# c5shen/WITCH

Measured on AMD Instinct MI355X. Metric: query-seqs aligned/sec (100k queries x 200-HMM eHMM), higher is better.
Workload: dtype f32; 1 GPU; dna_100k_x200; n_queries=100000, n_hmms=200, query_len=150, model_len_min=898, model_len_max=993, k=10, pairs_reported_rank0=20000000, pairs_multidomain_rank0=968, pairs_long_list_rank0=0, pairs_dense_redo_rank0=3, topk_crc32=3263627139

## Files before the change

include/witch_hip.h:

```cpp
#ifndef WITCH_HIP_H
#define WITCH_HIP_H

#include <stdint.h>

#ifdef __cplusplus
extern "C" {
#endif

#define WH_OK          0
#define WH_EINVAL     -1
#define WH_EIO        -2
#define WH_ENODEV     -3
#define WH_EHIP       -4
#define WH_ERANGE     -5
#define WH_ENOMEM     -6

#define WH_ALPH_DNA    0
#define WH_ALPH_RNA    1
#define WH_ALPH_AMINO  2

#define WH_FLAG_REPORTED  1
#define WH_FLAG_MULTI     2
#define WH_FLAG_OVERRIDE  4
#define WH_FLAG_TRUNC     8
// ... 113 lines not shown
int wh_filter_host(const char *const *hmm_paths, int n, const uint8_t *residues, const int64_t *offsets, int64_t nq,
                   const wh_filter_opts *opts, uint8_t *stage, float *filter_bias_nats, int32_t *msv_raw, int32_t *vit_raw,
                   int64_t *counts4);
int wh_score_filtered(wh_ehmm *e, const uint8_t *residues, const int64_t *offsets, int64_t nq, const wh_filter_opts *opts,
                      int32_t *decibits, uint8_t *flags, float *fwd_bits, wh_pair_detail *detail, uint8_t *stage);
int wh_score_filtered_dev(wh_ehmm *e, const uint8_t *d_residues, const int64_t *d_offsets, int64_t nq, int64_t total_residues,
                          int32_t max_len, const wh_filter_opts *opts, int32_t *d_decibits, uint8_t *d_flags, float *d_fwd_bits,
                          wh_pair_detail *d_detail, uint8_t *d_stage, void *stream);
int wh_last_filter_counts(wh_ehmm *e, int64_t out[6]);

int wh_last_align_status(wh_ehmm *e, int64_t *n_logspace, int64_t *n_unaligned, int64_t *unaligned_pairs, int64_t cap);

int wh_last_align_paths(wh_ehmm *e, int64_t *paths4);

int wh_last_score_paths(wh_ehmm *e, int64_t *paths6);
int wh_last_score_counters(wh_ehmm *e, int64_t *out8);
int wh_last_region_overflow(wh_ehmm *e, int64_t *out4);
int wh_last_long_query_pairs(wh_ehmm *e, int64_t out[2]);
int wh_last_long_score_pairs(wh_ehmm *e, int64_t out[2]);
int wh_last_long_align_pairs(wh_ehmm *e, int64_t out[2]);

int wh_set_path_buffer(wh_ehmm *e, uint8_t *d_paths);
int wh_set_path_buffer16(wh_ehmm *e, uint16_t *d_paths);

int wh_last_queue_reruns(wh_ehmm *e);

int wh_consensus(wh_ehmm *e, const int64_t *offsets, int64_t nq, const int64_t *qpair_off,
                 const int32_t *pair_h, const double *pair_w, const int64_t *col_offsets, const int32_t *cols,
                 const int64_t *ret_off, const int32_t *retained, const int32_t *nongaps,
                 int32_t backbone_length, int32_t *out, int32_t *minmax);
// ... 79 lines not shown
```

witch_amd/_lib.py:

```python
from __future__ import annotations

import ctypes as C
import os
import subprocess

_HERE = os.path.dirname(os.path.abspath(__file__))
LIB_PATH = os.path.join(_HERE, "libwitch_hip.so")
CSRC = os.path.join(_HERE, "csrc")

WH_MAX_ENVELOPES = 16
FLAG_REPORTED, FLAG_MULTI, FLAG_OVERRIDE, FLAG_TRUNC, FLAG_EXACT = 1, 2, 4, 8, 16
FLAG_FILTERED = 32
STAGE_MSV, STAGE_BIAS, STAGE_VIT, STAGE_VIT_RAN, STAGE_FWD = 1, 2, 4, 8, 16
VIT_NOT_RUN, VIT_OVERFLOW, MSV_OVERFLOW = -32769, 32768, -1
ALPH_DNA, ALPH_RNA, ALPH_AMINO = 0, 1, 2
WH_OK, WH_EINVAL, WH_EIO, WH_ENODEV, WH_EHIP, WH_ERANGE, WH_ENOMEM = 0, -1, -2, -3, -4, -5, -6
WH_BUILD_STATS, WH_BUILD_CALIB_NO_LDS = 1, 4
WH_MSA_TRIM, WH_MSA_NO_LDS, WH_MSA_CONS_HMMER = 1, 2, 4
PATH_P2_WIN, PATH_P2_FULL, PATH_P4_W256, PATH_P4_W512, PATH_P4_WFAIL, PATH_P4_FULL, PATH_DENSE, PATH_MULTI = 1, 2, 4, 8, 16, 32, 64, 128


class WitchHipError(RuntimeError):
    pass

# ... 88 lines not shown
                                  C.POINTER(C.c_void_p), C.POINTER(C.c_int64)] + [C.POINTER(C.c_void_p)] * 5 + [_P]),
    "wh_filter": (C.c_int, [_P, _P, _P, C.c_int64, _P, _P, _P, _P, _P]),
    "wh_filter_dev": (C.c_int, [_P, _P, _P, C.c_int64, C.c_int64, C.c_int32, _P, _P, _P, _P, _P, _P]),
    "wh_filter_host": (C.c_int, [C.POINTER(C.c_char_p), C.c_int, _P, _P, C.c_int64, _P, _P, _P, _P, _P, _P]),
    "wh_score_filtered": (C.c_int, [_P, _P, _P, C.c_int64, _P, _P, _P, _P, _P, _P]),
    "wh_score_filtered_dev": (C.c_int, [_P, _P, _P, C.c_int64, C.c_int64, C.c_int32, _P, _P, _P, _P, _P, _P, _P]),
    "wh_last_filter_counts": (C.c_int, [_P, _P]),
    "wh_ehmm_evparams": (C.c_int, [_P, _P, _P, _P]),
    "wh_hmm_evparams": (C.c_int, [C.c_char_p, C.POINTER(C.c_float), C.POINTER(C.c_float), C.POINTER(C.c_int32)]),
    "wh_consensus": (C.c_int, [_P, _P, C.c_int64, _P, _P, _P, _P, _P, _P, _P, _P, C.c_int32, _P, _P]),
    "wh_consensus_dev": (C.c_int, [_P, _P, C.c_int64, C.c_int32, _P, _P, _P, _P, _P, _P, _P, _P, C.c_int32, C.c_int32, _P, _P, _P]),
    "wh_last_align_status": (C.c_int, [_P, C.POINTER(C.c_int64), C.POINTER(C.c_int64), _P, C.c_int64]),
    "wh_last_align_paths": (C.c_int, [_P, _P]),
    "wh_last_score_paths": (C.c_int, [_P, _P]),
    "wh_last_score_counters": (C.c_int, [_P, _P]),
    "wh_set_path_buffer": (C.c_int, [_P, _P]),
    "wh_set_path_buffer16": (C.c_int, [_P, _P]),
    "wh_last_queue_reruns": (C.c_int, [_P]),
    "wh_last_region_overflow": (C.c_int, [_P, _P]),
    "wh_last_long_query_pairs": (C.c_int, [_P, _P]),
    "wh_last_long_score_pairs": (C.c_int, [_P, _P]),
    "wh_last_long_align_pairs": (C.c_int, [_P, _P]),
    "wh_last_score_launches": (C.c_int, [_P, _P, _P, _P, C.c_int]),
    "wh_last_kernel_ms": (C.c_int, [_P, C.c_int, C.POINTER(C.c_double), C.POINTER(C.c_int)]),
    "wh_set_timing": (C.c_int, [_P, C.c_int]),
    "wh_set_option": (C.c_int, [_P, C.c_char_p, C.c_char_p]),
}

_LIB = None

# ... 36 lines not shown
```

witch_amd/csrc/wh_api.hip:

```cpp
#include <atomic>
#include <chrono>
#include <memory>
#include <thread>

#include "wh_host.h"

static int g_device = -1;

extern "C" {

const char *wh_version(void) { return "witch_hip 0.1.0 (gfx950)"; }
const char *wh_last_error(void) { return wh::last_error(); }

int wh_init(int device) {
  int n = 0;
  if (hipGetDeviceCount(&n) != hipSuccess || n <= 0) {
    set_error("no HIP device visible");
    return WH_ENODEV;
  }
  if (device < 0 || device >= n) {
    set_error("device %d out of range (0..%d)", device, n - 1);
    return WH_EINVAL;
  }
  HIPCHK(hipSetDevice(device));
// ... 217 lines not shown

int wh_last_align_paths(wh_ehmm *e, int64_t *paths4) {
  if (!e || !paths4) { set_error("wh_last_align_paths: bad argument"); return WH_EINVAL; }
  for (int t = 0; t < 4; t++) paths4[t] = e->last_align_paths[t];
  return WH_OK;
}

int wh_last_score_paths(wh_ehmm *e, int64_t *paths6) {
  int64_t *paths4 = paths6;
  if (!e || !paths4) { set_error("wh_last_score_paths: bad argument"); return WH_EINVAL; }
  HIPCHK(hipSetDevice(e->device));
  unsigned long long v[6] = {0, 0, 0, 0, 0, 0};
  HIPCHK(hipDeviceSynchronize());
  HIPCHK(hipMemcpy(v, e->counter(kSlotScorePath), sizeof v, hipMemcpyDeviceToHost));
  for (int t = 0; t < 6; t++) paths4[t] = (int64_t)v[t];
  return WH_OK;
}

int wh_last_score_counters(wh_ehmm *e, int64_t *out8) {
  if (!e || !out8) { set_error("wh_last_score_counters: bad argument"); return WH_EINVAL; }
  HIPCHK(hipSetDevice(e->device));
  unsigned long long v[8] = {0, 0, 0, 0, 0, 0, 0, 0};
  HIPCHK(hipDeviceSynchronize());
  HIPCHK(hipMemcpy(v, e->counter(kSlotScorePath), sizeof v, hipMemcpyDeviceToHost));
  for (int t = 0; t < 8; t++) out8[t] = (int64_t)v[t];
  out8[7] = e->last_long_list;
  return WH_OK;
}

int wh_set_path_buffer(wh_ehmm *e, uint8_t *d_paths) {
  if (!e) { set_error("wh_set_path_buffer: null handle"); return WH_EINVAL; }
  e->path_buf = d_paths;
  return WH_OK;
}

int wh_set_path_buffer16(wh_ehmm *e, uint16_t *d_paths) {
  if (!e) { set_error("wh_set_path_buffer16: null handle"); return WH_EINVAL; }
  e->path_buf16 = d_paths;
  return WH_OK;
}
// ... 339 lines not shown
```

witch_amd/csrc/wh_host_score.hip:

```cpp
#include "wh_host.h"

static const int kStagedMaxBatches = 1 << 15;
static const int kStagedQB = 48;

static int resolve_main_cap(int max_M) {
  const size_t per_wave = (kLdsBudget - resolve_lds_header_bytes(0)) / (size_t)resolve_waves_per_cu();
  int lo = 1, hi = 1 << 20;
  while (lo < hi) {
    const int mid = lo + (hi - lo + 1) / 2;
    if (resolve_lds_bytes(mid, max_M) <= per_wave) lo = mid; else hi = mid - 1;
  }
  return lo;
}

static ScoreCall score_call(wh_ehmm *e, const uint8_t *d_residues, const int64_t *d_offsets, int64_t nq, int64_t total_residues, int32_t max_len,
                            int32_t *d_decibits, uint8_t *d_flags, float *d_fwd_bits, wh_pair_detail *d_detail, void *stream) {
  ScoreCall c = {e, (hipStream_t)stream, d_residues, d_offsets, nq, total_residues, max_len, d_decibits, d_flags, d_fwd_bits, d_detail};
  c.Lc = std::max(max_len, 1);
  c.H = (int)e->hmms.size();
  c.npairs_all = nq * (int64_t)c.H;
  const bool fits = resolve_lds_bytes(c.Lc, e->max_M) <= kLdsBudget;
  c.Lmain = fits || e->knobs.no_long_query ? c.Lc : resolve_main_cap(e->max_M);
  c.resolve = !e->knobs.no_resolve && (fits || !e->knobs.no_long_query) && c.npairs_all < 0x7FFFFFFF;
  c.mixed = nq > 0 && total_residues > 0 && (double)max_len > 1.25 * (double)total_residues / (double)nq;
// ... 97 lines not shown
static ScoreArgs class_args(const ScoreCall &c, const ScoreClassPlan &p, int launches) {
  const wh_ehmm *e = c.e;
  const Knobs &kn = e->knobs;
  ScoreArgs a;
  fill_common(a, c);
  a.tables = (const float *)e->d_tables.p;
  a.hmm_list = (const int32_t *)e->d_lists.p + p.list_off; a.n_list = p.n_list;
  a.counter = e->counter(kSlotLaunch0 + launches);
  a.dbg = kn.dbg;
  a.no_window = kn.no_window ? 1 : 0;
  a.keep_scale = kn.keep_scale;
  a.spill_band = kn.kernel != 9 ? kn.spill_band : 0;
  a.Klds = p.Klds; a.SP = p.b.SP; a.wave_lds = p.b.wave_lds; a.spec_arrays = kScoreSpecArrays;
  if (p.family == ScoreFamily::PhaseCall || p.family == ScoreFamily::FourEnvelope) a.spec_arrays |= kScoreSpecLayout << 8;
  a.paths = reinterpret_cast<unsigned long long *>(e->counter(kSlotScorePath));
  a.p2win = p.p2win;
  a.qorder = p.use_qorder ? c.d_qorder : nullptr;
  a.QB = p.QB; a.n_qblocks = p.n_qblocks; a.n_items = p.n_items;
  a.scratch_stride = p.scratch_stride; a.spec_stride = p.spec_stride;
  a.scratch = (float *)e->d_scratch.p;
  if (p.specg) a.spec_scratch = (float *)e->d_spec.p;
  return a;
}

static int print_class_stats(const ScoreCall &c, int Q, const unsigned long long *stats) {
  unsigned long long st[40];
  if (int rc = stats_read(c, stats, st)) return rc;
  const double tot = (double)(st[4] + st[5] + st[6] + st[7] + st[8] + st[9] + st[10] + st[11]);
  fprintf(stderr, "[wh] Q=%d wave cycles: P1 %.1f%%  P2 %.1f%%  regions %.1f%%  P3 %.1f%%  P4 %.1f%%  null2 %.1f%%  swaps+barriers %.1f%%  other %.1f%%  (total %.3g ticks)\n", Q, 100.0 * st[4] / tot,
          100.0 * st[5] / tot, 100.0 * st[6] / tot, 100.0 * st[7] / tot, 100.0 * st[8] / tot, 100.0 * st[9] / tot, 100.0 * st[10] / tot, 100.0 * st[11] / tot, tot);
  if (st[38]) fprintf(stderr, "[wh] Q=%d wave lifetimes %.3g cycles: %.1f%% in the phases above, %.1f%% fetching an item (two barriers)\n", Q, (double)st[38], 100.0 * tot / (double)st[38], 100.0 * (double)st[39] / (double)st[38]);
  if (st[37]) fprintf(stderr, "[wh] Q=%d four-envelope sweeps: %llu envelopes, %.0f wave cycles per envelope (slot 'null2' above)\n", Q, st[37], (double)st[9] / (double)st[37]);
  fprintf(stderr, "[wh] Q=%d envelope Backward sweeps: %llu on a 256-node window, %llu on a 512-node window, %llu windows failed the mass certificate, %llu full width; union of the stored lane blocks: span %.1f blocks (with margin), %.1f blocks set, of %llu envelopes\n", Q, st[0], st[1], st[2], st[3], (double)st[12] / (double)std::max(1ull, st[14]), (double)st[15] / (double)std::max(1ull, st[14]), st[14]);
  fprintf(stderr, "[wh] Q=%d multihit Backward on a window: %llu scans, of them in doubt at a threshold %llu, at the multidomain bound %llu; window loss out of range %llu; mean eps %.3g\n", Q,
          st[35], st[32], st[33], st[36], st[35] ? 1e-9 * (double)st[34] / (double)st[35] : 0.0);
  fprintf(stderr, "[wh] Q=%d |Ld - mass| / Ld  (<3e-7, <1e-6, <3e-6, <1e-5, <2e-5, more): window sweeps %llu %llu %llu %llu %llu %llu; full-width sweeps %llu %llu %llu %llu %llu %llu\n", Q,
          st[16], st[17], st[18], st[19], st[20], st[21], st[22], st[23], st[24], st[25], st[26], st[27]);
  return WH_OK;
}

static int launch_score_class(const ScoreCall &c, const ScoreClassPlan &p, int *launches) {
  wh_ehmm *e = c.e;
  hipStream_t s = c.s;
  const int Q = p.Q, waves = p.b.waves, threads = waves * kWave;
  const bool big = p.family == ScoreFamily::PassSync;
  ScoreArgs a = class_args(c, p, *launches);
  if (a.p2win == 2) {
    a.p2_backup_stride = (size_t)kScoreSpecArrays * a.SP;
    if (e->d_p2bak.ensure((size_t)p.blocks * waves * a.p2_backup_stride * sizeof(float))) return WH_ENOMEM;
    a.p2_backup = (float *)e->d_p2bak.p;
  }
  if (int rc = stats_begin(c, 320, 13, &a.stats)) return rc;
  if (e->knobs.trace) fprintf(stderr, "[wh] score Q=%d kernel=%s specg=%d waves=%d blocks=%d lds=%zu SP=%d wave_lds=%d items=%d Lcap=%d\n", Q,
                              kFamilyName[(int)p.family], (int)p.specg, waves, p.blocks, p.b.lds, a.SP, a.wave_lds, a.n_items, a.Lcap);
  HIPCHK(hipMemsetAsync(a.counter, 0, sizeof(int), s));
  if (class_mark(e, s, Q, big ? 1 : 0)) return WH_EHIP;
  hipError_t err = big ? launch_score_big(Q, a, p.blocks, threads, p.b.lds, s)
                   : p.family == ScoreFamily::TwoQuery ? launch_score9(Q, a, p.blocks, threads, p.b.lds, s)
                   : p.family == ScoreFamily::FourEnvelope ? launch_score7q(Q, a, p.blocks, threads, p.b.lds, s)
                   : p.family == ScoreFamily::PhaseCallB ? launch_score7b(Q, a, p.blocks, threads, p.b.lds, s)
                                                         : launch_score7(Q, a, p.blocks, threads, p.b.lds, s);
  if (err != hipSuccess) { set_error("score kernel launch (Q=%d) failed: %s", Q, hipGetErrorString(err)); return WH_EHIP; }
  (*launches)++;
  return a.stats ? print_class_stats(c, Q, a.stats) : WH_OK;
}

static int print_staged_stats(const ScoreCall &c, int Q, const unsigned long long *stats) {
// ... 355 lines not shown
```

witch_amd/csrc/wh_knobs.h:

```cpp
#pragma once
#include <algorithm>
#include <climits>
#include <cmath>
#include <cstdlib>
#include <cstring>

struct Knobs {
  int kernel = 7;
  float keep_scale = 0.f;
  int spill_band = 1;
  int max_waves = 0;
  bool force_specg = false;
  bool no_logspace = false;
  bool no_wide_align = false;
  bool no_window = false;
  bool no_p2win = false;
  bool no_long_list = false;
  bool no_big_region = false;
  bool no_long_query = false;
  bool no_resolve = false;
  int score_lmain = 0;
  bool no_long_score = false;
  bool longq_force = false;
  int rqueue_cap = 0;
  int item_g = 0;
  int st_units = 0;
  bool stats = false, trace = false;
  int dbg = 0;
  int rdbg = 0;
};

// ... 9 lines not shown
  {"WH_SCORE_KERNEL", true, [](Knobs &k, const char *v) { const int kv = *v ? atoi(v) : 7; if (kv < 7 || kv > 12) return false; k.kernel = kv; return true; }},
  {"WH_KEEP_LOG2", true, [](Knobs &k, const char *v) { k.keep_scale = *v ? ldexpf(1.0f, atoi(v)) : 0.f; return true; }},
  WH_KNOB_INT("WH_SPILL_BAND", false, spill_band, INT_MIN, INT_MAX, 1),
  WH_KNOB_INT("WH_MAX_WAVES", true, max_waves, 1, 16, 0),
  WH_KNOB_BOOL("WH_FORCE_SPECG", force_specg),
  WH_KNOB_BOOL("WH_NO_LOGSPACE", no_logspace),
  WH_KNOB_BOOL("WH_NO_RESOLVE", no_resolve),
  WH_KNOB_BOOL("WH_NO_LONG_LIST", no_long_list),
  WH_KNOB_BOOL("WH_NO_BIG_REGION", no_big_region),
  WH_KNOB_BOOL("WH_NO_LONG_QUERY", no_long_query),
  WH_KNOB_INT("WH_SCORE_LMAIN", true, score_lmain, 0, INT_MAX, 0),
  WH_KNOB_BOOL("WH_NO_LONG_SCORE", no_long_score),
  WH_KNOB_BOOL("WH_LONGQ_FORCE", longq_force),
  WH_KNOB_BOOL("WH_NO_WINDOW", no_window),
  WH_KNOB_BOOL("WH_NO_P2WIN", no_p2win),
  WH_KNOB_INT("WH_RQUEUE_CAP", true, rqueue_cap, 1, INT_MAX, 0),
  WH_KNOB_INT("WH_ITEM_G", true, item_g, 1, 1024, 0),
  WH_KNOB_INT("WH_ST_UNITS", true, st_units, 16, INT_MAX, 0),
  WH_KNOB_BOOL("WH_NO_WIDE_ALIGN", no_wide_align),
  WH_KNOB_BOOL("WH_STATS", stats),
  WH_KNOB_BOOL("WH_TRACE", trace),
  WH_KNOB_INT("WH_DBG", true, dbg, INT_MIN, INT_MAX, 0),
  WH_KNOB_INT("WH_RDBG", true, rdbg, INT_MIN, INT_MAX, 0),
};
#undef WH_KNOB_BOOL
#undef WH_KNOB_INT

static inline int set_knob(Knobs &k, const char *name, const char *value) {
  for (const KnobEntry &kn : kKnobs)
    if (!strcmp(name, kn.name)) return kn.apply(k, value ? value : "") ? 1 : -1;
// ... 3 lines not shown
```

witch_amd/csrc/wh_score7.hip:

```cpp
#include <hip/hip_runtime.h>

#include "wh_device.h"
#include "wh_launch.h"

#ifndef WH_K7NS
#define WH_K7NS k7
#define WH_K7LAUNCH launch_score7
#endif

namespace wh {
namespace WH_K7NS {


constexpr float kKeepScale7 = 5.9604645e-08f;
constexpr float kMassTol7 = 2e-5f;
constexpr float kWinTol7 = 3e-6f;
__device__ __forceinline__ float spill_tol(bool banded) { return banded ? kWinTol7 : kMassTol7; }
#ifndef WH_K7_MAXQP
#define WH_K7_MAXQP 0
#endif
constexpr int kMaxQP = WH_K7_MAXQP;
#ifdef WH_SLIM_SPEC
constexpr bool kSlim = true;
constexpr int kSpML = SP_B, kSpMH = SP_E, kSpArr = 6;
// ... 10 lines not shown
#ifndef WH_SPEC_ROWS
#define WH_SPEC_ROWS WH_K7_NEW_DEFAULT
#endif
#ifndef WH_UNI
#define WH_UNI WH_K7_NEW_DEFAULT
#endif
#ifndef WH_ROW_PAIRS
#define WH_ROW_PAIRS (WH_K7_NEW_DEFAULT ? 3 : 0)
#endif
#ifndef WH_SPLIT_SLACK
#define WH_SPLIT_SLACK 1
#endif
#ifndef WH_ROW_WAITS
#define WH_ROW_WAITS (WH_K7_NEW_DEFAULT ? 3 : 0)
#endif
constexpr int kLayout = WH_SPEC_ROWS ? SPEC_ROWS : SPEC_SOA;
constexpr bool kUni = WH_UNI != 0;
constexpr bool kRowPairs = ((WH_ROW_PAIRS) & 1) != 0, kUniArgs = ((WH_ROW_PAIRS) & 2) != 0, kSplitSlack = WH_SPLIT_SLACK != 0;
constexpr bool kDrain = ((WH_ROW_WAITS) & 1) != 0, kLateRequest = ((WH_ROW_WAITS) & 2) != 0;
static_assert(kLayout == SPEC_SOA || kSlim, "a row record has six words (WH_SLIM_SPEC)");
template <bool SG> using SpecOf = SpecAt<SG ? (int)SPEC_SOA : kLayout>;
constexpr int kSpecTag = kSpArr | (kLayout << 8);

__device__ __noinline__ static double dlog(double x) { return log(x); }
__device__ __noinline__ static double dexp(double x) { return exp(x); }
__device__ __forceinline__ float flogsum0_v7(float b) {
  const float mx = b > 0.f ? b : 0.f, mn = b > 0.f ? 0.f : b;
  if (mn == -INFINITY || (mx - mn) >= 15.7f) return mx;
  const int idx = (int)((mx - mn) * 1000.0f);
  return mx + (float)dlog(1.0 + dexp((double)-idx / 1000.0));
// ... 684 lines not shown
#pragma unroll
      for (int a = 0; a < BW_NARR; a++) T.v[a][p4] = bw4[a * Q4 * kWave + rev];
    }
  }
  const ScanC sc = scan_prepare(lane_product<QB, true>(T, BW_DD));
  const LdsF4 em4L((const float *)c.emL);
  const float4 *em4G = reinterpret_cast<const float4 *>((const float *)c.emG);
  float Mb[QB], Ib[QB];
#pragma unroll
  for (int p = 0; p < QB; p++) { Mb[p] = 0.f; Ib[p] = 0.f; }
  float xC = cm.move, xJ = 0.f, xN = 0.f, xB = 0.f;
  int eb = 0;
  float ratio = 0.f;
  int S_row = 0;
  float E_row = 0.f, B_row = 0.f;
  if (CARRY) { S_row = speci[at(SP_S, L)]; E_row = spec[at(SP_E, L)]; B_row = spec[at(SP_B, L)]; }
#pragma unroll 1
  for (int i = L; i >= 0; i--) {
    asm volatile("" ::: "memory");
    const int S_i = CARRY ? S_row : 0;
    const float E_i = CARRY ? E_row : 0.f, B_i = CARRY ? B_row : 0.f;
    int S_p = 0;
    float N_p = 0.f, J_p = 0.f, C_p = 0.f;
    if (CARRY) {
      const int ip = i >= 1 ? i - 1 : 0;
      S_p = speci[at(SP_S, ip)]; N_p = spec[at(SP_N, ip)]; J_p = spec[at(SP_J, ip)]; C_p = spec[at(SP_C, ip)];
      E_row = spec[at(SP_E, ip)]; B_row = spec[at(SP_B, ip)];
      S_row = S_p;
    }
    if (i < L) {
      const int x = __builtin_amdgcn_readfirstlane((int)seq[i]);
      float part = 0.f;
      auto emit = [&](auto em_ld) {
#pragma unroll
        for (int p4 = 0; p4 < B4; p4++) {
          const float4 E = T.v[BW_E][p4];
          const float4 O = em_ld(p4);
          Mb[4 * p4 + 0] *= O.w; part = fmaf(E.x, Mb[4 * p4 + 0], part);
          Mb[4 * p4 + 1] *= O.z; part = fmaf(E.y, Mb[4 * p4 + 1], part);
          Mb[4 * p4 + 2] *= O.y; part = fmaf(E.z, Mb[4 * p4 + 2], part);
          Mb[4 * p4 + 3] *= O.x; part = fmaf(E.w, Mb[4 * p4 + 3], part);
        }
      };
      if (x < Klds) emit([&](int p4) { return em4L[x * (Q * 16) + fwd[p4]]; });
      else {
        emit([&](int p4) { return em4G[(size_t)x * (Q * 16) + fwd[p4]]; });
// ... 15 lines not shown
      xB *= r; xJ *= r; xC *= r; xN *= r; xE *= r;
      eb += e;
    }
    const float s_i = ldexpf(invZ, (CARRY ? S_i : speci[at(SP_S, i)]) + eb - ef_L);
    const float pe = (CARRY ? E_i : spec[at(SP_E, i)]) * xE * s_i;
    const float pb = (CARRY ? B_i : spec[at(SP_B, i)]) * xB * s_i;
    float njc = 0.f;
    if (i >= 1) {
      const float s_p = ldexpf(invZ, (CARRY ? S_p : speci[at(SP_S, i, 1)]) + eb - ef_L);
      njc = (CARRY ? N_p : spec[at(SP_N, i, 1)]) * xN;
      njc = fmaf(CARRY ? J_p : spec[at(SP_J, i, 1)], xJ, njc);
      njc = fmaf(CARRY ? C_p : spec[at(SP_C, i, 1)], xC, njc);
      njc = njc * cm.loop * s_p;
    } else {
      ratio = (CARRY ? N_p : spec[at(SP_N, 0)]) * xN * s_i;
    }
    __builtin_amdgcn_wave_barrier();
    if (TMPG) { if (lane == 0) { gE[i] = pe; gB[i] = pb; gN[i] = njc; } }
    else if (lane == 0) {
      if (INPL) { specw[at(SP_E, i)] = pe; specw[at(SP_B, i)] = pb; specw[at(SP_N, i)] = njc; }
      else { tmp[i] = pe; tmp[SP + i] = pb; tmp[2 * SP + i] = njc; }
    }
    __builtin_amdgcn_wave_barrier();
  }
  WinDec o;
  o.eps = 1.0f - ratio;
  return o;
}

template <int TH, bool INPL = false, bool TMPG = false>
// ... 268 lines not shown
    slot = __shfl(slot, 0);
    if (slot < a.rcap && lane == 0) {
      ResolveRec *rr = a.rrecs + slot;
      rr->q = qi; rr->h = h; rr->fwdsc = fwdsc; rr->fwd_bits = fwd_bits_out; rr->nreg = nreg; rr->nenv = nenv;
      rr->multi_mask = multi_mask; rr->flags = flags;
      for (int e = 0; e < nenv; e++) { rr->ri[e] = regs[2 * e]; rr->rj[e] = regs[2 * e + 1]; rr->envsc[e] = envres[e]; rr->domcorr[e] = envres[WH_MAX_ENVELOPES + e]; }
    }
  } else assemble_score(L, Ld_tot, seqbias_sum, sum_score, sb2, fwdsc, nullsc, dp, flags, decibits);
  }
}

struct FrontState {
  float eps_prev, eps_prev2;
  unsigned n_pairs_h;
  unsigned n_p2w, n_p2rej;
};
template <int Q, int TH, bool SG, bool TMPG>
__device__ __forceinline__ RegOut score_regions(const ScoreArgs &a, const WaveCtx &c, uint8_t *seq, int *regs, int L, int lane, LenCfg cm, const FwdOut &f1,
                                                FrontState &fs, long long &t_last, glb_f *tmpg = nullptr) {
  const int SP = c.SP;
  bool saved = false;
  RegOut ro;
  bool have_ro = false;
  if constexpr (Q >= 8 && !SG) {
    const bool try_win = fminf(fs.eps_prev, fs.eps_prev2) * (float)L < 0.17f || (fs.n_pairs_h & 15) == 0;
    fs.n_pairs_h++;
    if ((a.p2win == 1 || TMPG) && !a.no_window && try_win) {
      const unsigned *su = reinterpret_cast<const unsigned *>((const float *)c.n2tab) + kUmSlot;
      const unsigned long long um = ((unsigned long long)su[1] << 32) | su[0];
      if (um != 0) {
        int lo = __builtin_ctzll(um), hi = 63 - __builtin_clzll(um);
        lo = lo > 1 ? lo - 2 : 0; hi = hi < 63 ? hi + 1 : 63;
        const int nodes = (hi - lo + 1) * Q;
        WinDec wd;
        wd.eps = 1.0f;
        if (TMPG && nodes <= (Q % 8 == 0 && Q > 8 ? 8 : 4) * kWave) {
          const float *spec = (const float *)c.spec;
          if (kLayout == SPEC_ROWS) {
            for (int u = lane; u < kSpArr * (L + 1); u += kWave) __builtin_nontemporal_store(spec[u], tmpg + u);
          } else {
            for (int arr = 0; arr < kSpArr; arr++)
              for (int u = lane; u <= L; u += kWave) __builtin_nontemporal_store(spec[arr * SP + u], tmpg + arr * SP + u);
          }
          saved = true;
        }
        if (nodes <= 4 * kWave) wd = sweep_backward_decode_win<4, Q, TH, TMPG, false, false>(c, (lds_u8 *)seq, L, cm, 1.0f / (f1.xC * cm.move), f1.ef, min((63 - hi) * Q, kWave * (Q - 4)));
        else if (Q % 8 == 0 && Q > 8 && nodes <= 8 * kWave) wd = sweep_backward_decode_win<(Q % 8 == 0 ? 8 : 4), Q, TH, TMPG, false, false>(c, (lds_u8 *)seq, L, cm, 1.0f / (f1.xC * cm.move), f1.ef, min((63 - hi) * Q, kWave * (Q - 8)));
        if (nodes <= (Q % 8 == 0 && Q > 8 ? 8 : 4) * kWave) { fs.eps_prev2 = fs.eps_prev; fs.eps_prev = fabsf(wd.eps); }
        if (wd.eps > -1e-4f && wd.eps < 0.01f) {
          ro = region_scan_cert<TH, TMPG, false>(c.spec, SP, L, (lds_i *)regs, lane, fmaxf(wd.eps, 0.f));
          have_ro = ((ro.flags >> 24) & 3) == 0;
          if (a.stats && lane == 0) {
            if ((ro.flags >> 24) & 1) atomicAdd(a.stats + 32, 1ull);
            if ((ro.flags >> 25) & 1) atomicAdd(a.stats + 33, 1ull);
            atomicAdd(a.stats + 34, (unsigned long long)(wd.eps * 1e9f));
            atomicAdd(a.stats + 35, 1ull);
          }
          ro.flags &= 0xFFFFFF;
        } else if (a.stats && lane == 0) atomicAdd(a.stats + 36, 1ull);
        if (have_ro) fs.n_p2w++; else fs.n_p2rej++;
      }
    }
  }
  if (!have_ro) {
    if (TMPG && saved) {
      __builtin_amdgcn_fence(__ATOMIC_SEQ_CST, "workgroup");
      float *spec = (float *)c.spec;
      __builtin_amdgcn_wave_barrier();
      if (kLayout == SPEC_ROWS) {
        for (int u = lane; u < kSpArr * (L + 1); u += kWave) spec[u] = __builtin_nontemporal_load(tmpg + u);
      } else {
        for (int arr = 0; arr < kSpArr; arr++)
          for (int u = lane; u <= L; u += kWave) spec[arr * SP + u] = __builtin_nontemporal_load(tmpg + arr * SP + u);
      }
      __builtin_amdgcn_wave_barrier();
// ... 26 lines not shown

template <int Q, int TH, bool SG>
__global__ __launch_bounds__(TH) void score_kernel7(ScoreArgs a) {
  extern __shared__ __attribute__((aligned(16))) float smem_raw[];
  volatile int *s_item_p = reinterpret_cast<volatile int *>(smem_raw);
  float *smem = smem_raw + 4;
  const int lane = threadIdx.x & 63, wave = __builtin_amdgcn_readfirstlane((int)(threadIdx.x >> 6)), nwaves = blockDim.x >> 6;
  constexpr int TBL = Q * kWave;
  float *emL = smem;
  float *trL = smem + (size_t)a.K * TBL;
  constexpr int NARR = FW_NARR + (Q <= kMaxQP ? 1 : 0);
  float *wbase = trL + 2 * NARR * TBL + (size_t)wave * a.wave_lds;
  const int SP = a.SP;
  WaveCtx c;
  c.emL = (lds_f *)emL; c.fwL = (lds_f *)trL; c.bwL = (lds_f *)(trL + NARR * TBL);
  const int spArrAll = kSpArr + (a.p2win == 1 ? 3 : 0);
  c.spec = (lds_f *)wbase; c.n2tab = (lds_f *)(wbase + (SG ? 0 : spArrAll * SP));
  c.specg = SG ? (glb_f *)(a.spec_scratch + ((size_t)blockIdx.x * nwaves + wave) * a.spec_stride) : nullptr;
  c.degen = 0;
  for (int t = 0; t < 32; t++) if (t == lane) c.degen = a.degen[t];
  c.Fs = (glb_f *)(a.scratch + ((size_t)blockIdx.x * nwaves + wave) * a.scratch_stride);
  c.SP = SP; c.alpha = a.K | (a.Kp << 8) | (a.K << 16); c.lane = lane;
  int *regs = reinterpret_cast<int *>(wbase + (SG ? 0 : spArrAll * SP) + 32);
  uint8_t *seq = reinterpret_cast<uint8_t *>(regs + kRegsInts);
  const double LOG2 = 0.69314718055994529;
  int cur_h = -1;
  const DevHMM *hm = nullptr;
  EnvCounters ec = {0, 0, 0, 0, 0};
  FrontState fs = {0.f, 0.f, 0u, 0u, 0u};

  for (;;) {
    __syncthreads();
    if (threadIdx.x == 0) { *s_item_p = atomicAdd(a.counter, 1); s_item_p[1] = 0; }
    __syncthreads();
    const int item = __builtin_amdgcn_readfirstlane(*s_item_p);
    if (item >= a.n_items) break;
    const int h = __builtin_amdgcn_readfirstlane(a.hmm_list[item / a.n_qblocks]);
    const int64_t q_lo = (int64_t)(item % a.n_qblocks) * a.QB;
    const int64_t q_hi = q_lo + a.QB < a.nq ? q_lo + a.QB : a.nq;
    if (h != cur_h) {
      hm = a.hmms + h;
      const float4 *src = reinterpret_cast<const float4 *>(a.tables + hm->em_off);
      float4 *dst = reinterpret_cast<float4 *>(emL);
      for (int t = threadIdx.x; t < a.K * TBL / 4; t += blockDim.x) dst[t] = src[t];
// ... 60 lines not shown
        a.flags[out] = (uint8_t)flags;
        if (a.fwd_bits) a.fwd_bits[out] = fwd_bits_out;
      }
      const unsigned band_ev = take_band_events(ec);
      if (uint16_t *rec = path_record(a)) {
        if (lane == 0) rec[out] = (uint16_t)path_bits(regs, ec, fs, isfinite(fwd_bits_out), flags, (flags & WH_FLAG_MULTI) && a.rrecs != nullptr, band_ev);
      }
    }
  }
  if (a.paths && lane == 0) {
    if (ec.n_w256) atomicAdd(a.paths + 0, (unsigned long long)ec.n_w256);
    if (ec.n_w512) atomicAdd(a.paths + 1, (unsigned long long)ec.n_w512);
    if (ec.n_wfail) atomicAdd(a.paths + 2, (unsigned long long)ec.n_wfail);
    if (ec.n_full) atomicAdd(a.paths + 3, (unsigned long long)ec.n_full);
    if (ec.spill) atomicAdd(a.paths + 6, ec.spill);
    if (fs.n_p2w) atomicAdd(a.paths + 4, (unsigned long long)fs.n_p2w);
    if (fs.n_p2rej) atomicAdd(a.paths + 5, (unsigned long long)fs.n_p2rej);
  }
}

enum { QR_QLO = 0, QR_QHI, QR_L, QR_NREG, QR_FLAGS, QR_FWDSC, QR_NULLSC, QR_FWDBITS, QR_ENVSC, QR_RI, QR_RJ, QR_XC3, QR_EF3, QR_BAND, QR_INTS = 16 };
template <int Q, int TH>
__global__ __launch_bounds__(TH) void score_kernel7q(ScoreArgs a) {
  extern __shared__ __attribute__((aligned(16))) float smem_raw[];
  volatile int *s_item_p = reinterpret_cast<volatile int *>(smem_raw);
  float *smem = smem_raw + 4;
  const int lane = threadIdx.x & 63, wave = threadIdx.x >> 6, nwaves = blockDim.x >> 6;
  constexpr int TBL = Q * kWave;
  float *emL = smem;
  float *trL = smem + (size_t)a.K * TBL;
  float *wbase = trL + 2 * FW_NARR * TBL + (size_t)wave * a.wave_lds;
// ... 10 lines not shown
  c.degen = 0;
  for (int t = 0; t < 32; t++) if (t == lane) c.degen = a.degen[t];
  const int slab1 = (int)(a.scratch_stride / 5);
  glb_f *Fs0 = (glb_f *)(a.scratch + wid * a.scratch_stride) + slab1;
  glb_f *FsW = Fs0 - slab1;
  c.Fs = FsW;
  c.SP = SP; c.alpha = a.K | (a.Kp << 8) | (a.K << 16); c.lane = lane;
  int *regs = reinterpret_cast<int *>(wbase + kSpArr * SP + 128);
  int *qslots = regs + kRegsInts;
  int *qrecs = qslots + 4 * QS_INTS;
  uint8_t *seqs = reinterpret_cast<uint8_t *>(qrecs + 4 * QR_INTS);
  const double LOG2 = 0.69314718055994529;
  int cur_h = -1;
  const DevHMM *hm = nullptr;
  EnvCounters ec = {0, 0, 0, 0, 0};
  FrontState fs = {0.f, 0.f, 0u, 0u, 0u};
  const long long t_kernel0 = a.stats ? (long long)__builtin_readcyclecounter() : 0;

  for (;;) {
    const long long t_bar0 = a.stats ? (long long)__builtin_readcyclecounter() : 0;
    __syncthreads();
    if (threadIdx.x == 0) { *s_item_p = atomicAdd(a.counter, 1); s_item_p[1] = 0; }
    __syncthreads();
    const int item = *s_item_p;
    if (a.stats && lane == 0) atomicAdd(a.stats + 39, (unsigned long long)((long long)__builtin_readcyclecounter() - t_bar0));
    if (item >= a.n_items) break;
    const int h = a.hmm_list[item / a.n_qblocks];
    const int64_t q_lo = (int64_t)(item % a.n_qblocks) * a.QB;
    const int64_t q_hi = q_lo + a.QB < a.nq ? q_lo + a.QB : a.nq;
    if (h != cur_h) {
      hm = a.hmms + h;
// ... 186 lines not shown
          if (dp) { dp->env_i[0] = ri; dp->env_j[0] = rj; dp->envsc[0] = envsc; dp->domcorr[0] = domcorr; }
          assemble_score(L, Ld_tot, domcorr, sum_score, sb2, fwdsc, nullsc, dp, flags, decibits);
          if (lane == 0) { a.decibits[out] = decibits; a.flags[out] = (uint8_t)flags; }
        }
        WH_TICK7(11);
      }
    }
  }
  (void)take_band_events(ec);
  if (a.paths && lane == 0) {
    if (ec.n_w256) atomicAdd(a.paths + 0, (unsigned long long)ec.n_w256);
    if (ec.n_w512) atomicAdd(a.paths + 1, (unsigned long long)ec.n_w512);
    if (ec.n_wfail) atomicAdd(a.paths + 2, (unsigned long long)ec.n_wfail);
    if (ec.n_full) atomicAdd(a.paths + 3, (unsigned long long)ec.n_full);
    if (ec.spill) atomicAdd(a.paths + 6, ec.spill);
    if (fs.n_p2w) atomicAdd(a.paths + 4, (unsigned long long)fs.n_p2w);
    if (fs.n_p2rej) atomicAdd(a.paths + 5, (unsigned long long)fs.n_p2rej);
  }
  if (a.stats && lane == 0) atomicAdd(a.stats + 38, (unsigned long long)(__builtin_readcyclecounter() - t_kernel0));
}

template <int Q, int TH>
static hipError_t launch7q(const ScoreArgs &a, int blocks, int threads, size_t lds, hipStream_t s) {
  hipError_t err = hipFuncSetAttribute(reinterpret_cast<const void *>(&score_kernel7q<Q, TH>), hipFuncAttributeMaxDynamicSharedMemorySize, (int)lds);
  if (err != hipSuccess) return err;
  hipLaunchKernelGGL((score_kernel7q<Q, TH>), dim3(blocks), dim3(threads), lds, s, a);
  return hipGetLastError();
}

template <int Q, int TH, bool SG>
static hipError_t launch7sg(const ScoreArgs &a, int blocks, int threads, size_t lds, hipStream_t s) {
// ... 49 lines not shown
```

witch_amd/ehmm.py:

```python
from __future__ import annotations

import ctypes as C

import numpy as np

from . import _lib
from ._lib import DOMAIN_FIELDS, FilterOpts, PairDetail, WitchHipError, check, lib


def pack_queries(seqs):
    offs = np.zeros(len(seqs) + 1, dtype=np.int64)
    if len(seqs):
        offs[1:] = np.cumsum([len(s) for s in seqs])
        res = np.concatenate([np.asarray(s, dtype=np.uint8) for s in seqs])
    else:
        res = np.zeros(0, dtype=np.uint8)
    return np.ascontiguousarray(res), offs


def alignment_checksum(molecule, rows):
    rows = [r.encode() if isinstance(r, str) else bytes(r) for r in rows]
    if not rows or len(set(len(r) for r in rows)) != 1:
        raise ValueError("alignment_checksum: the rows must be of one length")
    out = C.c_uint32(0)
# ... 71 lines not shown
        ms, n = C.c_double(0), C.c_int(0)
        check(lib().wh_last_kernel_ms(self._h, which, C.byref(ms), C.byref(n)), "wh_last_kernel_ms")
        return ms.value, n.value

    def last_score_launches(self):
        q = np.zeros(64, dtype=np.int32)
        kind = np.zeros(64, dtype=np.int32)
        ms = np.zeros(64, dtype=np.float64)
        n = lib().wh_last_score_launches(self._h, q.ctypes.data, kind.ctypes.data, ms.ctypes.data, 64)
        check(min(n, 0), "wh_last_score_launches")
        return [(int(q[t]), int(kind[t]), float(ms[t])) for t in range(min(n, 64))]

    def last_score_paths(self):
        p6 = np.zeros(6, dtype=np.int64)
        check(lib().wh_last_score_paths(self._h, p6.ctypes.data), "wh_last_score_paths")
        return {"window256": int(p6[0]), "window512": int(p6[1]), "window_rejected": int(p6[2]), "full_width": int(p6[3]),
                "p2_window": int(p6[4]), "p2_window_in_doubt": int(p6[5])}

    def last_score_spill_bytes(self) -> int:
        c8 = np.zeros(8, dtype=np.int64)
        check(lib().wh_last_score_counters(self._h, c8.ctypes.data), "wh_last_score_counters")
        return int(c8[6])

    def last_long_list_pairs(self) -> int:
        c8 = np.zeros(8, dtype=np.int64)
        check(lib().wh_last_score_counters(self._h, c8.ctypes.data), "wh_last_score_counters")
        return int(c8[7])

    def last_region_overflow(self):
        o4 = np.zeros(4, dtype=np.int64)
        check(lib().wh_last_region_overflow(self._h, o4.ctypes.data), "wh_last_region_overflow")
        return {"pairs": int(o4[0]), "max_domains": int(o4[1]), "max_segments": int(o4[2]), "max_clusters": int(o4[3])}
# ... 435 lines not shown
```

Before: 25580 queries/s.

## Add 512-node window escalation after doubt and batch P2 tmp row stores per wave

```diff
diff --git a/include/witch_hip.h b/include/witch_hip.h
--- a/include/witch_hip.h
+++ b/include/witch_hip.h
@@ -151,6 +151,7 @@
 int wh_last_align_paths(wh_ehmm *e, int64_t *paths4);
 
 int wh_last_score_paths(wh_ehmm *e, int64_t *paths6);
+int wh_last_score_p2_escalated(wh_ehmm *e, int64_t *out1);
 int wh_last_score_counters(wh_ehmm *e, int64_t *out8);
 int wh_last_region_overflow(wh_ehmm *e, int64_t *out4);
 int wh_last_long_query_pairs(wh_ehmm *e, int64_t out[2]);
diff --git a/witch_amd/_lib.py b/witch_amd/_lib.py
--- a/witch_amd/_lib.py
+++ b/witch_amd/_lib.py
@@ -126,6 +126,7 @@
     "wh_last_align_paths": (C.c_int, [_P, _P]),
     "wh_last_score_paths": (C.c_int, [_P, _P]),
     "wh_last_score_counters": (C.c_int, [_P, _P]),
+    "wh_last_score_p2_escalated": (C.c_int, [_P, _P]),
     "wh_set_path_buffer": (C.c_int, [_P, _P]),
     "wh_set_path_buffer16": (C.c_int, [_P, _P]),
     "wh_last_queue_reruns": (C.c_int, [_P]),
diff --git a/witch_amd/csrc/wh_api.hip b/witch_amd/csrc/wh_api.hip
--- a/witch_amd/csrc/wh_api.hip
+++ b/witch_amd/csrc/wh_api.hip
@@ -255,6 +255,17 @@
   HIPCHK(hipDeviceSynchronize());
   HIPCHK(hipMemcpy(v, e->counter(kSlotScorePath), sizeof v, hipMemcpyDeviceToHost));
   for (int t = 0; t < 6; t++) paths4[t] = (int64_t)v[t];
+  paths4[4] = (int64_t)(v[4] & 0xFFFFFFFFull);
+  return WH_OK;
+}
+
+int wh_last_score_p2_escalated(wh_ehmm *e, int64_t *out1) {
+  if (!e || !out1) { set_error("wh_last_score_p2_escalated: bad argument"); return WH_EINVAL; }
+  HIPCHK(hipSetDevice(e->device));
+  unsigned long long v = 0;
+  HIPCHK(hipDeviceSynchronize());
+  HIPCHK(hipMemcpy(&v, reinterpret_cast<unsigned long long *>(e->counter(kSlotScorePath)) + 4, sizeof v, hipMemcpyDeviceToHost));
+  *out1 = (int64_t)(v >> 32);
   return WH_OK;
 }
 
@@ -265,6 +276,7 @@
   HIPCHK(hipDeviceSynchronize());
   HIPCHK(hipMemcpy(v, e->counter(kSlotScorePath), sizeof v, hipMemcpyDeviceToHost));
   for (int t = 0; t < 8; t++) out8[t] = (int64_t)v[t];
+  out8[4] = (int64_t)(v[4] & 0xFFFFFFFFull);
   out8[7] = e->last_long_list;
   return WH_OK;
 }
diff --git a/witch_amd/csrc/wh_host_score.hip b/witch_amd/csrc/wh_host_score.hip
--- a/witch_amd/csrc/wh_host_score.hip
+++ b/witch_amd/csrc/wh_host_score.hip
@@ -135,7 +135,7 @@
   a.Klds = p.Klds; a.SP = p.b.SP; a.wave_lds = p.b.wave_lds; a.spec_arrays = kScoreSpecArrays;
   if (p.family == ScoreFamily::PhaseCall || p.family == ScoreFamily::FourEnvelope) a.spec_arrays |= kScoreSpecLayout << 8;
   a.paths = reinterpret_cast<unsigned long long *>(e->counter(kSlotScorePath));
-  a.p2win = p.p2win;
+  a.p2win = p.p2win | (p.p2win == 1 && kn.p2_escalate ? 4 : 0);
   a.qorder = p.use_qorder ? c.d_qorder : nullptr;
   a.QB = p.QB; a.n_qblocks = p.n_qblocks; a.n_items = p.n_items;
   a.scratch_stride = p.scratch_stride; a.spec_stride = p.spec_stride;
@@ -145,7 +145,7 @@
 }
 
 static int print_class_stats(const ScoreCall &c, int Q, const unsigned long long *stats) {
-  unsigned long long st[40];
+  unsigned long long st[56];
   if (int rc = stats_read(c, stats, st)) return rc;
   const double tot = (double)(st[4] + st[5] + st[6] + st[7] + st[8] + st[9] + st[10] + st[11]);
   fprintf(stderr, "[wh] Q=%d wave cycles: P1 %.1f%%  P2 %.1f%%  regions %.1f%%  P3 %.1f%%  P4 %.1f%%  null2 %.1f%%  swaps+barriers %.1f%%  other %.1f%%  (total %.3g ticks)\n", Q, 100.0 * st[4] / tot,
@@ -155,6 +155,11 @@
   fprintf(stderr, "[wh] Q=%d envelope Backward sweeps: %llu on a 256-node window, %llu on a 512-node window, %llu windows failed the mass certificate, %llu full width; union of the stored lane blocks: span %.1f blocks (with margin), %.1f blocks set, of %llu envelopes\n", Q, st[0], st[1], st[2], st[3], (double)st[12] / (double)std::max(1ull, st[14]), (double)st[15] / (double)std::max(1ull, st[14]), st[14]);
   fprintf(stderr, "[wh] Q=%d multihit Backward on a window: %llu scans, of them in doubt at a threshold %llu, at the multidomain bound %llu; window loss out of range %llu; mean eps %.3g\n", Q,
           st[35], st[32], st[33], st[36], st[35] ? 1e-9 * (double)st[34] / (double)st[35] : 0.0);
+  if (st[28]) {
+    auto p95 = [&](int b0) { unsigned long long n = 0; int b = 0; for (; b < 8; b++) { n += st[b0 + b]; if (20 * n >= 19 * st[28]) break; } return ldexp(1.0, std::min(b, 7) - 13); };
+    fprintf(stderr, "[wh] Q=%d multihit Backward, 512-node window after a doubt: %llu scans, %llu certified (%.1f%%); mean eps %.3g on 256 nodes -> %.3g on 512; 95%% of them below %.3g -> %.3g (powers of two, 2^-6: or more)\n", Q,
+            st[28], st[29], 100.0 * (double)st[29] / (double)st[28], 1e-9 * (double)st[30] / (double)st[28], 1e-9 * (double)st[31] / (double)st[28], p95(40), p95(48));
+  }
   fprintf(stderr, "[wh] Q=%d |Ld - mass| / Ld  (<3e-7, <1e-6, <3e-6, <1e-5, <2e-5, more): window sweeps %llu %llu %llu %llu %llu %llu; full-width sweeps %llu %llu %llu %llu %llu %llu\n", Q,
           st[16], st[17], st[18], st[19], st[20], st[21], st[22], st[23], st[24], st[25], st[26], st[27]);
   return WH_OK;
@@ -166,12 +171,12 @@
   const int Q = p.Q, waves = p.b.waves, threads = waves * kWave;
   const bool big = p.family == ScoreFamily::PassSync;
   ScoreArgs a = class_args(c, p, *launches);
-  if (a.p2win == 2) {
+  if ((a.p2win & 3) == 2) {
     a.p2_backup_stride = (size_t)kScoreSpecArrays * a.SP;
     if (e->d_p2bak.ensure((size_t)p.blocks * waves * a.p2_backup_stride * sizeof(float))) return WH_ENOMEM;
     a.p2_backup = (float *)e->d_p2bak.p;
   }
-  if (int rc = stats_begin(c, 320, 13, &a.stats)) return rc;
+  if (int rc = stats_begin(c, 448, 13, &a.stats)) return rc;
   if (e->knobs.trace) fprintf(stderr, "[wh] score Q=%d kernel=%s specg=%d waves=%d blocks=%d lds=%zu SP=%d wave_lds=%d items=%d Lcap=%d\n", Q,
                               kFamilyName[(int)p.family], (int)p.specg, waves, p.blocks, p.b.lds, a.SP, a.wave_lds, a.n_items, a.Lcap);
   HIPCHK(hipMemsetAsync(a.counter, 0, sizeof(int), s));
diff --git a/witch_amd/csrc/wh_knobs.h b/witch_amd/csrc/wh_knobs.h
--- a/witch_amd/csrc/wh_knobs.h
+++ b/witch_amd/csrc/wh_knobs.h
@@ -15,6 +15,7 @@
   bool no_wide_align = false;
   bool no_window = false;
   bool no_p2win = false;
+  bool p2_escalate = false;
   bool no_long_list = false;
   bool no_big_region = false;
   bool no_long_query = false;
@@ -54,6 +55,7 @@
   WH_KNOB_BOOL("WH_LONGQ_FORCE", longq_force),
   WH_KNOB_BOOL("WH_NO_WINDOW", no_window),
   WH_KNOB_BOOL("WH_NO_P2WIN", no_p2win),
+  WH_KNOB_BOOL("WH_P2_ESCALATE", p2_escalate),
   WH_KNOB_INT("WH_RQUEUE_CAP", true, rqueue_cap, 1, INT_MAX, 0),
   WH_KNOB_INT("WH_ITEM_G", true, item_g, 1, 1024, 0),
   WH_KNOB_INT("WH_ST_UNITS", true, st_units, 16, INT_MAX, 0),
diff --git a/witch_amd/csrc/wh_score7.hip b/witch_amd/csrc/wh_score7.hip
--- a/witch_amd/csrc/wh_score7.hip
+++ b/witch_amd/csrc/wh_score7.hip
@@ -48,6 +48,10 @@
 #ifndef WH_ROW_WAITS
 #define WH_ROW_WAITS (WH_K7_NEW_DEFAULT ? 3 : 0)
 #endif
+#ifndef WH_P2_ROWS64
+#define WH_P2_ROWS64 (WH_K7_NEW_DEFAULT ? 3 : 0)
+#endif
+constexpr bool kP2Rows64 = ((WH_P2_ROWS64) & 1) != 0, kP2SeqAhead = ((WH_P2_ROWS64) & 2) != 0;
 constexpr int kLayout = WH_SPEC_ROWS ? SPEC_ROWS : SPEC_SOA;
 constexpr bool kUni = WH_UNI != 0;
 constexpr bool kRowPairs = ((WH_ROW_PAIRS) & 1) != 0, kUniArgs = ((WH_ROW_PAIRS) & 2) != 0, kSplitSlack = WH_SPLIT_SLACK != 0;
@@ -762,6 +766,10 @@
   float ratio = 0.f;
   int S_row = 0;
   float E_row = 0.f, B_row = 0.f;
+  constexpr bool R64 = kP2Rows64 && !INPL && !TMPG;
+  float ve = 0.f, vb = 0.f, vn = 0.f;
+  constexpr bool XA = kP2SeqAhead && !INPL && !TMPG;
+  int x_row = 0;
   if (CARRY) { S_row = speci[at(SP_S, L)]; E_row = spec[at(SP_E, L)]; B_row = spec[at(SP_B, L)]; }
 #pragma unroll 1
   for (int i = L; i >= 0; i--) {
@@ -776,8 +784,10 @@
       E_row = spec[at(SP_E, ip)]; B_row = spec[at(SP_B, ip)];
       S_row = S_p;
     }
+    const int x_i = x_row;
+    if (XA) x_row = (int)seq[i >= 1 ? i - 1 : 0];
     if (i < L) {
-      const int x = __builtin_amdgcn_readfirstlane((int)seq[i]);
+      const int x = __builtin_amdgcn_readfirstlane(XA ? x_i : (int)seq[i]);
       float part = 0.f;
       auto emit = [&](auto em_ld) {
 #pragma unroll
@@ -823,6 +833,19 @@
       njc = njc * cm.loop * s_p;
     } else {
       ratio = (CARRY ? N_p : spec[at(SP_N, 0)]) * xN * s_i;
+    }
+    if (R64) {
+      const bool mine = lane == (i & (kWave - 1));
+      ve = mine ? pe : ve; vb = mine ? pb : vb; vn = mine ? njc : vn;
+      if ((i & (kWave - 1)) == 0) {
+        __builtin_amdgcn_wave_barrier();
+        int r0 = i;
+        asm volatile("" : "+s"(r0));
+        const int r = r0 + lane;
+        if (r <= L) { tmp[r] = ve; tmp[SP + r] = vb; tmp[2 * SP + r] = vn; }
+        __builtin_amdgcn_wave_barrier();
+      }
+      continue;
     }
     __builtin_amdgcn_wave_barrier();
     if (TMPG) { if (lane == 0) { gE[i] = pe; gB[i] = pb; gN[i] = njc; } }
@@ -1121,6 +1144,7 @@
   float eps_prev, eps_prev2;
   unsigned n_pairs_h;
   unsigned n_p2w, n_p2rej;
+  unsigned n_p2esc;
 };
 template <int Q, int TH, bool SG, bool TMPG>
 __device__ __forceinline__ RegOut score_regions(const ScoreArgs &a, const WaveCtx &c, uint8_t *seq, int *regs, int L, int lane, LenCfg cm, const FwdOut &f1,
@@ -1132,7 +1156,7 @@
   if constexpr (Q >= 8 && !SG) {
     const bool try_win = fminf(fs.eps_prev, fs.eps_prev2) * (float)L < 0.17f || (fs.n_pairs_h & 15) == 0;
     fs.n_pairs_h++;
-    if ((a.p2win == 1 || TMPG) && !a.no_window && try_win) {
+    if (((a.p2win & 3) == 1 || TMPG) && !a.no_window && try_win) {
       const unsigned *su = reinterpret_cast<const unsigned *>((const float *)c.n2tab) + kUmSlot;
       const unsigned long long um = ((unsigned long long)su[1] << 32) | su[0];
       if (um != 0) {
@@ -1151,21 +1175,40 @@
           }
           saved = true;
         }
-        if (nodes <= 4 * kWave) wd = sweep_backward_decode_win<4, Q, TH, TMPG, false, false>(c, (lds_u8 *)seq, L, cm, 1.0f / (f1.xC * cm.move), f1.ef, min((63 - hi) * Q, kWave * (Q - 4)));
-        else if (Q % 8 == 0 && Q > 8 && nodes <= 8 * kWave) wd = sweep_backward_decode_win<(Q % 8 == 0 ? 8 : 4), Q, TH, TMPG, false, false>(c, (lds_u8 *)seq, L, cm, 1.0f / (f1.xC * cm.move), f1.ef, min((63 - hi) * Q, kWave * (Q - 8)));
-        if (nodes <= (Q % 8 == 0 && Q > 8 ? 8 : 4) * kWave) { fs.eps_prev2 = fs.eps_prev; fs.eps_prev = fabsf(wd.eps); }
-        if (wd.eps > -1e-4f && wd.eps < 0.01f) {
-          ro = region_scan_cert<TH, TMPG, false>(c.spec, SP, L, (lds_i *)regs, lane, fmaxf(wd.eps, 0.f));
-          have_ro = ((ro.flags >> 24) & 3) == 0;
-          if (a.stats && lane == 0) {
-            if ((ro.flags >> 24) & 1) atomicAdd(a.stats + 32, 1ull);
-            if ((ro.flags >> 25) & 1) atomicAdd(a.stats + 33, 1ull);
-            atomicAdd(a.stats + 34, (unsigned long long)(wd.eps * 1e9f));
-            atomicAdd(a.stats + 35, 1ull);
-          }
-          ro.flags &= 0xFFFFFF;
-        } else if (a.stats && lane == 0) atomicAdd(a.stats + 36, 1ull);
-        if (have_ro) fs.n_p2w++; else fs.n_p2rej++;
+        constexpr int QW = Q % 8 == 0 && Q > 8 ? 8 : 4;
+        constexpr bool ESC = QW == 8 && !TMPG && !(Q == 16 && TH == 512);
+        int qb = nodes <= 4 * kWave ? 4 : nodes <= QW * kWave ? QW : 0;
+        bool second = false;
+        while (qb != 0) {
+          if (qb == 4) wd = sweep_backward_decode_win<4, Q, TH, TMPG, false, false>(c, (lds_u8 *)seq, L, cm, 1.0f / (f1.xC * cm.move), f1.ef, min((63 - hi) * Q, kWave * (Q - 4)));
+          else if constexpr (QW == 8) wd = sweep_backward_decode_win<QW, Q, TH, TMPG, false, false>(c, (lds_u8 *)seq, L, cm, 1.0f / (f1.xC * cm.move), f1.ef, min((63 - hi) * Q, kWave * (Q - 8)));
+          qb = 0;
+          if (wd.eps > -1e-4f && wd.eps < 0.01f) {
+            ro = region_scan_cert<TH, TMPG, false>(c.spec, SP, L, (lds_i *)regs, lane, fmaxf(wd.eps, 0.f));
+            have_ro = ((ro.flags >> 24) & 3) == 0;
+            if (a.stats && lane == 0) {
+              if ((ro.flags >> 24) & 1) atomicAdd(a.stats + 32, 1ull);
+              if ((ro.flags >> 25) & 1) atomicAdd(a.stats + 33, 1ull);
+              atomicAdd(a.stats + 34, (unsigned long long)(wd.eps * 1e9f));
+              atomicAdd(a.stats + 35, 1ull);
+              if (second) {
+                atomicAdd(a.stats + 28, 1ull);
+                if (have_ro) atomicAdd(a.stats + 29, 1ull);
+                atomicAdd(a.stats + 30, (unsigned long long)(fabsf(fs.eps_prev) * 1e9f));
+                atomicAdd(a.stats + 31, (unsigned long long)(wd.eps * 1e9f));
+                atomicAdd(a.stats + 40 + min(max(f32_exponent(fmaxf(fabsf(fs.eps_prev), 1e-30f)) + 14, 0), 7), 1ull);
+                atomicAdd(a.stats + 48 + min(max(f32_exponent(fmaxf(wd.eps, 1e-30f)) + 14, 0), 7), 1ull);
+              }
+            }
+            ro.flags &= 0xFFFFFF;
+            if (ESC && !have_ro && !second && (a.p2win & 4) != 0 && nodes <= 4 * kWave) { qb = QW; second = true; fs.eps_prev2 = fs.eps_prev; fs.eps_prev = fabsf(wd.eps); }
+          } else if (a.stats && lane == 0) atomicAdd(a.stats + 36, 1ull);
+        }
+        if (nodes <= QW * kWave) {
+          if (second) fs.eps_prev = fabsf(wd.eps);
+          else { fs.eps_prev2 = fs.eps_prev; fs.eps_prev = fabsf(wd.eps); }
+        }
+        if (have_ro) { if (second) fs.n_p2esc++; else fs.n_p2w++; } else fs.n_p2rej++;
       }
     }
   }
@@ -1222,7 +1265,7 @@
   const int SP = a.SP;
   WaveCtx c;
   c.emL = (lds_f *)emL; c.fwL = (lds_f *)trL; c.bwL = (lds_f *)(trL + NARR * TBL);
-  const int spArrAll = kSpArr + (a.p2win == 1 ? 3 : 0);
+  const int spArrAll = kSpArr + ((a.p2win & 3) == 1 ? 3 : 0);
   c.spec = (lds_f *)wbase; c.n2tab = (lds_f *)(wbase + (SG ? 0 : spArrAll * SP));
   c.specg = SG ? (glb_f *)(a.spec_scratch + ((size_t)blockIdx.x * nwaves + wave) * a.spec_stride) : nullptr;
   c.degen = 0;
@@ -1235,7 +1278,7 @@
   int cur_h = -1;
   const DevHMM *hm = nullptr;
   EnvCounters ec = {0, 0, 0, 0, 0};
-  FrontState fs = {0.f, 0.f, 0u, 0u, 0u};
+  FrontState fs = {0.f, 0.f, 0u, 0u, 0u, 0u};
 
   for (;;) {
     __syncthreads();
@@ -1326,7 +1369,7 @@
     if (ec.n_wfail) atomicAdd(a.paths + 2, (unsigned long long)ec.n_wfail);
     if (ec.n_full) atomicAdd(a.paths + 3, (unsigned long long)ec.n_full);
     if (ec.spill) atomicAdd(a.paths + 6, ec.spill);
-    if (fs.n_p2w) atomicAdd(a.paths + 4, (unsigned long long)fs.n_p2w);
+    if (fs.n_p2w | fs.n_p2esc) atomicAdd(a.paths + 4, (unsigned long long)fs.n_p2w | ((unsigned long long)fs.n_p2esc << 32));
     if (fs.n_p2rej) atomicAdd(a.paths + 5, (unsigned long long)fs.n_p2rej);
   }
 }
@@ -1367,7 +1410,7 @@
   int cur_h = -1;
   const DevHMM *hm = nullptr;
   EnvCounters ec = {0, 0, 0, 0, 0};
-  FrontState fs = {0.f, 0.f, 0u, 0u, 0u};
+  FrontState fs = {0.f, 0.f, 0u, 0u, 0u, 0u};
   const long long t_kernel0 = a.stats ? (long long)__builtin_readcyclecounter() : 0;
 
   for (;;) {
@@ -1584,7 +1627,7 @@
     if (ec.n_wfail) atomicAdd(a.paths + 2, (unsigned long long)ec.n_wfail);
     if (ec.n_full) atomicAdd(a.paths + 3, (unsigned long long)ec.n_full);
     if (ec.spill) atomicAdd(a.paths + 6, ec.spill);
-    if (fs.n_p2w) atomicAdd(a.paths + 4, (unsigned long long)fs.n_p2w);
+    if (fs.n_p2w | fs.n_p2esc) atomicAdd(a.paths + 4, (unsigned long long)fs.n_p2w | ((unsigned long long)fs.n_p2esc << 32));
     if (fs.n_p2rej) atomicAdd(a.paths + 5, (unsigned long long)fs.n_p2rej);
   }
   if (a.stats && lane == 0) atomicAdd(a.stats + 38, (unsigned long long)(__builtin_readcyclecounter() - t_kernel0));
diff --git a/witch_amd/ehmm.py b/witch_amd/ehmm.py
--- a/witch_amd/ehmm.py
+++ b/witch_amd/ehmm.py
@@ -109,8 +109,10 @@
     def last_score_paths(self):
         p6 = np.zeros(6, dtype=np.int64)
         check(lib().wh_last_score_paths(self._h, p6.ctypes.data), "wh_last_score_paths")
+        esc = np.zeros(1, dtype=np.int64)
+        check(lib().wh_last_score_p2_escalated(self._h, esc.ctypes.data), "wh_last_score_p2_escalated")
         return {"window256": int(p6[0]), "window512": int(p6[1]), "window_rejected": int(p6[2]), "full_width": int(p6[3]),
-                "p2_window": int(p6[4]), "p2_window_in_doubt": int(p6[5])}
+                "p2_window": int(p6[4]), "p2_window_in_doubt": int(p6[5]), "p2_window_512_after_doubt": int(esc[0])}
 
     def last_score_spill_bytes(self) -> int:
         c8 = np.zeros(8, dtype=np.int64)
```

Result: no change. 25660 queries/s, median of 6 (+0.3%).
